# eliasandronicou/split-learning-k8s

Hardware: AMD Instinct MI355X
Metric: training samples/sec (node) for split CNN (higher is better)
Workload: dtype fp32; 1 GPU; K2: split CNN (model_def.py ModelPartA+ModelPartB) both stages fused on 1xMI355X, synthetic 1x28x28 MNIST-shape batches, fp32, HIP-graph step; global_batch=4096, per_gpu_batch=4096, topology=fused-1gpu, graph=True, conv=x3, cut_handoff=client conv1 writes the x3 split input images (slk_conv1_fwd_x3); no f32 cut, client_backward=fused into the x3 dgrad (slk_conv2_dgrad_x3_c1w); no cut gradient in HBM

## Files before the change

include/slk.h:

```cpp
#ifndef SLK_H
#define SLK_H

#include <stdint.h>

#ifdef __cplusplus
extern "C" {
#endif

#define SLK_ABI_VERSION 1

#define SLK_CLIENT_NPARAM 320
#define SLK_SERVER_NPARAM 110666
#define SLK_OFF_W2 0
#define SLK_OFF_B2 18432
#define SLK_OFF_W3 18496
#define SLK_OFF_B3 110656

int slk_abi_version(void);
const char* slk_error_string(int err);
const char* slk_build_id(void);


int slk_conv1_fwd(const float* x, const float* W1, const float* b1, float* act, int B, void* stream);

int slk_conv1_fwd_amax(const float* x, const float* W1, const float* b1, float* act, float* act_amax, int B,
                       void* stream);

int slk_conv1_wgrad(const float* x, const float* act, const float* cut_grad, float* slabs, int B,
                    void* stream);
int slk_conv1_wgrad_nslab(int B);
int slk_conv1_wgrad_remask(const float* x, const float* W1, const float* b1, const float* cut_grad, float* slabs,
                           int B, void* stream);


int slk_conv2_fwd_pool(const float* act, const float* W2, const float* b2, float* pooled,
                       uint8_t* code, int B, void* stream);
int slk_conv2_fwd_pool_direct(const float* act, const float* W2, const float* b2, float* pooled,
                              uint8_t* code, int B, void* stream);

int slk_fc_fwd(const float* pooled, const float* W3, const float* b3, float* logits, int B,
               void* stream);

int slk_xent_fwd_bwd(const float* logits, const int64_t* labels, float* loss_i, float* dlogits,
                     float grad_scale, int* err_flag, int B, void* stream);

int slk_fc_logits_xent(const float* pooled, const float* W3, const float* b3, const int64_t* labels, float* logits,
                       float* loss_i, float* dlogits, float grad_scale, int* err_flag, int B, void* stream);

int slk_fc_dgrad(const float* dlogits, const float* W3, float* dpooled, int B, void* stream);
int slk_fc_dgrad_amax(const float* dlogits, const float* W3, float* dpooled, float* dp_amax, int B, void* stream);

int slk_fc_xent(const float* pooled, const float* W3, const float* b3, const int64_t* labels,
                float* logits, float* loss_i, float* dlogits, float* dpooled, float grad_scale,
                int* err_flag, int B, void* stream);

int slk_fc_xent_amax(const float* pooled, const float* W3, const float* b3, const int64_t* labels, float* logits,
                     float* loss_i, float* dlogits, float* dpooled, float* dp_amax, float grad_scale, int* err_flag,
                     int B, void* stream);


int slk_xent_soft_fwd_bwd(const float* logits, const int64_t* labels, float* loss_i, float* dlogits, float grad_scale,
                          float smoothing, int* err_flag, int B, void* stream);
int slk_fc_logits_xent_soft(const float* pooled, const float* W3, const float* b3, const int64_t* labels,
                            float* logits, float* loss_i, float* dlogits, float grad_scale, float smoothing,
                            int* err_flag, int B, void* stream);
int slk_fc_xent_soft(const float* pooled, const float* W3, const float* b3, const int64_t* labels, float* logits,
                     float* loss_i, float* dlogits, float* dpooled, float* dp_amax, float grad_scale, float smoothing,
                     int* err_flag, int B, void* stream);

int slk_fc_wgrad(const float* dlogits, const float* pooled, float* slabs, int B, void* stream);
int slk_fc_wgrad_nslab(int B);

int slk_conv2_dgrad(const float* dpooled, const uint8_t* code, const float* W2, float* cut_grad,
                    int B, void* stream);
int slk_conv2_dgrad_direct(const float* dpooled, const uint8_t* code, const float* W2, float* cut_grad,
                           int B, void* stream);

int slk_conv2_wgrad(const float* act, const float* dpooled, const uint8_t* code, float* slabs,
                    int B, void* stream);
int slk_conv2_wgrad_nslab(int B);
int slk_conv2_wgrad_direct(const float* act, const float* dpooled, const uint8_t* code, float* slabs,
                           int B, void* stream);
int slk_conv2_wgrad_direct_nslab(int B);


int slk_row_amax(const float* x, int rows, int n, float* amax, void* stream);
int slk_conv2_fwd_pool_x3(const float* act, const float* act_amax, const float* W2, const float* b2, float* pooled,
                          uint8_t* code, int B, void* stream);
int slk_conv2_dgrad_x3(const float* dpooled, const float* dp_amax, const uint8_t* code, const float* W2,
                       float* cut_grad, int B, void* stream);
int slk_conv2_wgrad_x3(const float* act, const float* act_amax, const float* dpooled, const float* dp_amax,
                       const uint8_t* code, float* slabs, int B, void* stream);
int slk_conv2_wgrad_x3_nslab(int B);
int slk_conv2_fwd_pool_x3s(const float* act, const float* act_amax, const float* W2, const float* b2, float* pooled,
                           uint8_t* code, uint16_t* act16, int B, void* stream);
int slk_conv2_wgrad_x3s(const uint16_t* act16, const float* act_amax, const float* dpooled, const float* dp_amax,
                        const uint8_t* code, float* slabs, int B, void* stream);
int slk_conv2_wgrad_x3_form(void);
int slk_mfma_probe_blocks(void);
int slk_mfma_probe(float* out, int iters, void* stream);
int slk_conv2_fwd_pool_x3sa(const float* act, float* act_amax, const float* W2, const float* b2, float* pooled,
                            uint8_t* code, uint16_t* act16, int B, void* stream);
int64_t slk_conv2_act16_bytes(int B);

int slk_conv1_fwd_x3(const float* x, const float* W1, const float* b1, float* act, float* act_amax, uint16_t* act16,
                     uint32_t* relu_bits, int B, void* stream);
int64_t slk_relu_bits_bytes(int B);
int slk_conv2_fwd_pool_x3i(const uint16_t* act16, const float* act_amax, const float* W2, const float* b2,
                           float* pooled, uint8_t* code, int B, void* stream);

int slk_conv2_fwd_pool_x3p(const uint16_t* act16, const float* act_amax, const float* W2, const float* b2,
                           float* pooled, int B, void* stream);

int slk_conv2_dgrad_x3_c1w(const float* dpooled, const float* dp_amax, const uint8_t* code, const float* W2,
                           const float* x, const uint32_t* relu_bits, float* client_slabs, int B, void* stream);
int slk_conv2_dgrad_x3_c1w_nslab(int B);


int slk_fc_eval(const float* pooled, const float* W3, const float* b3, const int64_t* labels, float* logits,
                float* loss_i, int64_t* pred, int* err_flag, int B, void* stream);

int slk_eval_logits(const float* logits, const int64_t* labels, int B, float* loss_i, int64_t* pred, int* err_flag,
                    void* stream);

// ... 171 lines not shown
```

split-learning-k8s_amd/csrc/slk_server.hip:

```cpp
#include "slk_common.h"
#include "slk_eval.h"

using namespace slk;

constexpr int C2F_WAVES = 12;
constexpr int C2F_THREADS = C2F_WAVES * 64;
constexpr int C2F_IMG = 16 * A_PIX;
constexpr int C2F_WH = 72 * 2 * 64;
constexpr int C2F_TPW = 3;
constexpr int C2F_GRID = 256;
constexpr int C2F_CHUNKS = (C2F_IMG * 4 + 1023) / 1024;

typedef __attribute__((address_space(3))) void* lds_ptr_t;

__device__ __forceinline__ void c2f_dma_half(const float* __restrict__ src, float* dst, int wave, int lane) {
    const char* s = reinterpret_cast<const char*>(src);
    char* d = reinterpret_cast<char*>(dst);
    for (int c = wave; c < C2F_CHUNKS; c += C2F_WAVES) {
        const int off = c * 1024 + lane * 16;
        if (off < C2F_IMG * 4)
            __builtin_amdgcn_global_load_lds((const void*)(s + off), (lds_ptr_t)(d + c * 1024), 16, 0, 0);
    }
}

// ... 596 lines not shown
        __syncthreads();
    }

    if constexpr ((MODE & 4) != 0) {
        const float4* W34 = reinterpret_cast<const float4*>(W3);
        float4* D4 = reinterpret_cast<float4*>(dpooled + (size_t)s0 * P_SAMPLE);
        float dmx[FCH_S];
#pragma unroll
        for (int s = 0; s < FCH_S; ++s) dmx[s] = 0.f;
        for (int k4 = tid; k4 < FC_K4; k4 += FCH_T) {
            asm volatile("" ::: "memory");
            float4 w[NCLS];
#pragma unroll
            for (int jj = 0; jj < NCLS; ++jj) w[jj] = W34[jj * FC_K4 + k4];
#pragma unroll
            for (int s = 0; s < FCH_S; ++s) {
                if (s < ns) {
                    float4 o = make_float4(0.f, 0.f, 0.f, 0.f);
#pragma unroll
                    for (int jj = 0; jj < NCLS; ++jj) {
                        const float d = dl[s][jj];
                        o.x = fmaf(d, w[jj].x, o.x);
                        o.y = fmaf(d, w[jj].y, o.y);
                        o.z = fmaf(d, w[jj].z, o.z);
                        o.w = fmaf(d, w[jj].w, o.w);
                    }
                    D4[s * FC_K4 + k4] = o;
                    dmx[s] = fmaxf(dmx[s], fmaxf(fmaxf(fabsf(o.x), fabsf(o.y)), fmaxf(fabsf(o.z), fabsf(o.w))));
                }
            }
        }
        if (dp_amax) {
#pragma unroll
            for (int s = 0; s < FCH_S; ++s) {
                const float v = wave_max(dmx[s]);
                if (lane == 0) mx[wave][s] = v;
            }
            __syncthreads();
            if (tid < ns) {
                float v = mx[0][tid];
#pragma unroll
                for (int w = 1; w < FCH_W; ++w) v = fmaxf(v, mx[w][tid]);
                dp_amax[s0 + tid] = v;
            }
        }
    }
}

#ifndef SLK_FCW_MAXSPLIT
#define SLK_FCW_MAXSPLIT 64
#endif
constexpr int FCW_MAXSPLIT = SLK_FCW_MAXSPLIT;
constexpr int FCW_SLAB = W3_N + NCLS;
__global__ __launch_bounds__(256) void fc_wgrad_kernel(const float* __restrict__ dlogits,
                                                       const float* __restrict__ pooled,
                                                       float* __restrict__ slabs, int B, int per) {
    const int k4 = blockIdx.x * 256 + threadIdx.x;
    const int sp = blockIdx.y;
    const int bs = sp * per, be = min(B, bs + per);
    float4 acc[NCLS];
#pragma unroll
    for (int jj = 0; jj < NCLS; ++jj) acc[jj] = make_float4(0.f, 0.f, 0.f, 0.f);
    const float4* P4 = reinterpret_cast<const float4*>(pooled);
    int b = bs;
    for (; b + 8 <= be; b += 8) {
        float4 p[8];
#pragma unroll
        for (int u = 0; u < 8; ++u) p[u] = P4[(size_t)(b + u) * FC_K4 + k4];
#pragma unroll
        for (int u = 0; u < 8; ++u)
#pragma unroll
            for (int jj = 0; jj < NCLS; ++jj) {
                const float d = dlogits[(b + u) * NCLS + jj];
                acc[jj].x = fmaf(d, p[u].x, acc[jj].x); acc[jj].y = fmaf(d, p[u].y, acc[jj].y);
                acc[jj].z = fmaf(d, p[u].z, acc[jj].z); acc[jj].w = fmaf(d, p[u].w, acc[jj].w);
            }
    }
    for (; b < be; ++b) {
        const float4 p = P4[(size_t)b * FC_K4 + k4];
#pragma unroll
        for (int jj = 0; jj < NCLS; ++jj) {
            const float d = dlogits[b * NCLS + jj];
            acc[jj].x = fmaf(d, p.x, acc[jj].x); acc[jj].y = fmaf(d, p.y, acc[jj].y);
            acc[jj].z = fmaf(d, p.z, acc[jj].z); acc[jj].w = fmaf(d, p.w, acc[jj].w);
        }
    }
    float* slab = slabs + (size_t)sp * FCW_SLAB;
#pragma unroll
    for (int jj = 0; jj < NCLS; ++jj) reinterpret_cast<float4*>(slab + jj * P_SAMPLE)[k4] = acc[jj];
    if (blockIdx.x == 0 && threadIdx.x < NCLS) {
        float s = 0.f;
        for (int bb = bs; bb < be; ++bb) s += dlogits[bb * NCLS + threadIdx.x];
        slab[W3_N + threadIdx.x] = s;
    }
}

static inline int fcw_per(int B) {
    int ns = (B + 63) / 64;
    if (ns > FCW_MAXSPLIT) ns = FCW_MAXSPLIT;
    if (ns < 1) ns = 1;
    return (B + ns - 1) / ns;
}
extern "C" int slk_fc_wgrad_nslab(int B) {
    if (B <= 0) return 0;
    const int per = fcw_per(B);
    return (B + per - 1) / per;
}

extern "C" int slk_conv2_fwd_pool_direct(const float* act, const float* W2, const float* b2, float* pooled,
                                  uint8_t* code, int B, void* stream) {
    SLK_CHECK_ARG(B >= 0);
    if (B == 0) return 0;
    SLK_CHECK_ARG(act && W2 && b2 && pooled && code);
    conv2_fwd_pool_kernel<<<B < C2F_GRID ? B : C2F_GRID, C2F_THREADS, 0, slk_stream(stream)>>>(
        act, W2, b2, pooled, code, B);
    return slk_launch_status();
}

extern "C" int slk_conv2_dgrad_direct(const float* dpooled, const uint8_t* code, const float* W2,
                               float* cut_grad, int B, void* stream) {
    SLK_CHECK_ARG(B >= 0);
    if (B == 0) return 0;
    SLK_CHECK_ARG(dpooled && code && W2 && cut_grad);
    conv2_dgrad_kernel<<<B < C2D_GRID ? B : C2D_GRID, C2D_THREADS, 0, slk_stream(stream)>>>(
        dpooled, code, W2, cut_grad, B);
    return slk_launch_status();
}

extern "C" int slk_conv2_wgrad_direct(const float* act, const float* dpooled, const uint8_t* code,
                               float* slabs, int B, void* stream) {
    SLK_CHECK_ARG(B >= 0);
    if (B == 0) return 0;
    SLK_CHECK_ARG(act && dpooled && code && slabs);
    conv2_wgrad_kernel<<<slk_conv2_wgrad_direct_nslab(B), C2W_THREADS, 0, slk_stream(stream)>>>(
        act, dpooled, code, slabs, B);
    return slk_launch_status();
}

extern "C" int slk_fc_fwd(const float* pooled, const float* W3, const float* b3, float* logits,
                          int B, void* stream) {
    SLK_CHECK_ARG(B >= 0);
    if (B == 0) return 0;
    SLK_CHECK_ARG(pooled && W3 && b3 && logits);
    fc_head16_kernel<1><<<(B + FCH_S - 1) / FCH_S, FCH_T, 0, slk_stream(stream)>>>(
        pooled, W3, b3, nullptr, logits, nullptr, nullptr, nullptr, 0.f, nullptr, B, nullptr);
    return slk_launch_status();
}

extern "C" int slk_xent_fwd_bwd(const float* logits, const int64_t* labels, float* loss_i,
                                float* dlogits, float grad_scale, int* err_flag, int B, void* stream) {
    SLK_CHECK_ARG(B >= 0);
    if (B == 0) return 0;
    SLK_CHECK_ARG(logits && labels && loss_i && dlogits);
    fc_head16_kernel<2><<<(B + FCH_S - 1) / FCH_S, FCH_T, 0, slk_stream(stream)>>>(
        nullptr, nullptr, nullptr, labels, const_cast<float*>(logits), loss_i, dlogits, nullptr,
        grad_scale, err_flag, B, nullptr);
    return slk_launch_status();
}

extern "C" int slk_fc_logits_xent(const float* pooled, const float* W3, const float* b3, const int64_t* labels,
                                  float* logits, float* loss_i, float* dlogits, float grad_scale, int* err_flag, int B,
// ... 58 lines not shown
    fc_head16_kernel<7><<<(B + FCH_S - 1) / FCH_S, FCH_T, 0, slk_stream(stream)>>>(
        pooled, W3, b3, labels, logits, loss_i, dlogits, dpooled, grad_scale, err_flag, B, dp_amax);
    return slk_launch_status();
}

#define SLK_CHECK_SMOOTHING(e) SLK_CHECK_ARG((e) >= 0.f && (e) <= 1.f)

extern "C" int slk_xent_soft_fwd_bwd(const float* logits, const int64_t* labels, float* loss_i, float* dlogits,
                                     float grad_scale, float smoothing, int* err_flag, int B, void* stream) {
    SLK_CHECK_ARG(B >= 0);
    SLK_CHECK_SMOOTHING(smoothing);
    if (B == 0) return 0;
    SLK_CHECK_ARG(logits && labels && loss_i && dlogits);
    fc_head16_kernel<2, true><<<(B + FCH_S - 1) / FCH_S, FCH_T, 0, slk_stream(stream)>>>(
        nullptr, nullptr, nullptr, labels, const_cast<float*>(logits), loss_i, dlogits, nullptr, grad_scale, err_flag, B,
        nullptr, nullptr, smoothing);
    return slk_launch_status();
}

extern "C" int slk_fc_logits_xent_soft(const float* pooled, const float* W3, const float* b3, const int64_t* labels,
                                       float* logits, float* loss_i, float* dlogits, float grad_scale, float smoothing,
                                       int* err_flag, int B, void* stream) {
    SLK_CHECK_ARG(B >= 0);
    SLK_CHECK_SMOOTHING(smoothing);
    if (B == 0) return 0;
    SLK_CHECK_ARG(pooled && W3 && b3 && labels && logits && loss_i && dlogits);
    fc_head16_kernel<3, true><<<(B + FCH_S - 1) / FCH_S, FCH_T, 0, slk_stream(stream)>>>(
        pooled, W3, b3, labels, logits, loss_i, dlogits, nullptr, grad_scale, err_flag, B, nullptr, nullptr, smoothing);
    return slk_launch_status();
}

extern "C" int slk_fc_xent_soft(const float* pooled, const float* W3, const float* b3, const int64_t* labels,
                                float* logits, float* loss_i, float* dlogits, float* dpooled, float* dp_amax,
                                float grad_scale, float smoothing, int* err_flag, int B, void* stream) {
    SLK_CHECK_ARG(B >= 0);
    SLK_CHECK_SMOOTHING(smoothing);
    if (B == 0) return 0;
    SLK_CHECK_ARG(pooled && W3 && b3 && labels && logits && loss_i && dlogits && dpooled);
    fc_head16_kernel<7, true><<<(B + FCH_S - 1) / FCH_S, FCH_T, 0, slk_stream(stream)>>>(
        pooled, W3, b3, labels, logits, loss_i, dlogits, dpooled, grad_scale, err_flag, B, dp_amax, nullptr, smoothing);
    return slk_launch_status();
}

extern "C" int slk_fc_wgrad(const float* dlogits, const float* pooled, float* slabs, int B,
                            void* stream) {
    SLK_CHECK_ARG(B >= 0);
    if (B == 0) return 0;
    SLK_CHECK_ARG(dlogits && pooled && slabs);
    const int per = fcw_per(B);
    dim3 grid(FC_K4 / 256, (B + per - 1) / per);
    fc_wgrad_kernel<<<grid, 256, 0, slk_stream(stream)>>>(dlogits, pooled, slabs, B, per);
    return slk_launch_status();
}
```

split-learning-k8s_amd/splitcnn/_lib.py:

```python
from __future__ import annotations

import ctypes
import os

import torch

from .build import CSRC_DIR, LIB_PATH, source_hash

_c_float_p = ctypes.c_void_p
_P = ctypes.c_void_p
_I = ctypes.c_int
_F = ctypes.c_float
_U = ctypes.c_uint
_L = ctypes.c_int64

_SIGS = {
    "slk_abi_version": [],
    "slk_cut_blocks": [_L],
    "slk_cut_encode": [_P, _L, _P, _P, _P, _P, _P, _P],
    "slk_cut_offsets": [_P, _L, _P, _P, _P, _P],
    "slk_cut_pack": [_P, _L, _P, _P, _P, _P],
    "slk_cut_unpack": [_P, _L, _P, _P, _P, _P],
    "slk_cut_ranks": [_P, _L, _P, _P, _P],
    "slk_cut_unpack_x3": [_P, _P, _P, _P, _I, _P, _P],
    "slk_conv2_dgrad_x3_pack": [_P, _P, _P, _P, _P, _P, _P, _I, _P],
    "slk_cut_offsets_ranks_parts": [_P, _I, _L, _P],
    "slk_cut_unpack_x3_parts": [_P, _I, _P, _I, _P, _P],
    "slk_conv2_dgrad_x3_pack_parts": [_P, _P, _P, _P, _P, _I, _I, _P],
    "slk_error_string": [_I],
    "slk_build_id": [],
    "slk_conv1_fwd": [_P, _P, _P, _P, _I, _P],
    "slk_conv1_fwd_amax": [_P, _P, _P, _P, _P, _I, _P],
    "slk_conv1_wgrad": [_P, _P, _P, _P, _I, _P],
    "slk_conv1_wgrad_nslab": [_I],
    "slk_conv1_wgrad_remask": [_P, _P, _P, _P, _P, _I, _P],
    "slk_conv2_fwd_pool": [_P, _P, _P, _P, _P, _I, _P],
    "slk_conv2_fwd_pool_direct": [_P, _P, _P, _P, _P, _I, _P],
    "slk_fc_fwd": [_P, _P, _P, _P, _I, _P],
    "slk_xent_fwd_bwd": [_P, _P, _P, _P, _F, _P, _I, _P],
    "slk_fc_logits_xent": [_P, _P, _P, _P, _P, _P, _P, _F, _P, _I, _P],
    "slk_fc_dgrad": [_P, _P, _P, _I, _P],
    "slk_fc_dgrad_amax": [_P, _P, _P, _P, _I, _P],
    "slk_fc_xent": [_P, _P, _P, _P, _P, _P, _P, _P, _F, _P, _I, _P],
    "slk_fc_xent_amax": [_P, _P, _P, _P, _P, _P, _P, _P, _P, _F, _P, _I, _P],
    "slk_xent_soft_fwd_bwd": [_P, _P, _P, _P, _F, _F, _P, _I, _P],
    "slk_fc_logits_xent_soft": [_P, _P, _P, _P, _P, _P, _P, _F, _F, _P, _I, _P],
    "slk_fc_xent_soft": [_P, _P, _P, _P, _P, _P, _P, _P, _P, _F, _F, _P, _I, _P],
    "slk_wide_head_soft": [_P, _P, _P, _P, _P, _U, _U, _F, _F, _F, _P, _P, _P, _P, _P, _P, _P, _I, _I, _P],
    "slk_image_batch_mix": [_P, _P, _I, _I, _I, _I, _P, _P, _I, _P, _P, _I, _I, _U, _U, ctypes.c_double, _P, _P, _P,
                            _P],
    "slk_fc_wgrad": [_P, _P, _P, _I, _P],
    "slk_fc_wgrad_nslab": [_I],
    "slk_conv2_dgrad": [_P, _P, _P, _P, _I, _P],
    "slk_conv2_dgrad_direct": [_P, _P, _P, _P, _I, _P],
    "slk_conv2_wgrad": [_P, _P, _P, _P, _I, _P],
    "slk_conv2_wgrad_nslab": [_I],
    "slk_conv2_wgrad_direct": [_P, _P, _P, _P, _I, _P],
    "slk_conv2_wgrad_direct_nslab": [_I],
    "slk_row_amax": [_P, _I, _I, _P, _P],
    "slk_conv2_fwd_pool_x3": [_P, _P, _P, _P, _P, _P, _I, _P],
    "slk_conv2_dgrad_x3": [_P, _P, _P, _P, _P, _I, _P],
    "slk_conv2_wgrad_x3": [_P, _P, _P, _P, _P, _P, _I, _P],
    "slk_conv2_wgrad_x3_nslab": [_I],
    "slk_conv2_fwd_pool_x3s": [_P, _P, _P, _P, _P, _P, _P, _I, _P],
    "slk_conv2_fwd_pool_x3sa": [_P, _P, _P, _P, _P, _P, _P, _I, _P],
    "slk_mfma_probe": [_P, _I, _P],
    "slk_mfma_probe_blocks": [],
    "slk_conv2_wgrad_x3s": [_P, _P, _P, _P, _P, _P, _I, _P],
    "slk_conv2_wgrad_x3_form": [],
    "slk_conv2_act16_bytes": [_I],
    "slk_conv1_fwd_x3": [_P, _P, _P, _P, _P, _P, _P, _I, _P],
    "slk_relu_bits_bytes": [_I],
    "slk_conv2_fwd_pool_x3i": [_P, _P, _P, _P, _P, _P, _I, _P],
    "slk_conv2_fwd_pool_x3p": [_P, _P, _P, _P, _P, _I, _P],
    "slk_fc_eval": [_P, _P, _P, _P, _P, _P, _P, _P, _I, _P],
    "slk_eval_logits": [_P, _P, _I, _P, _P, _P, _P],
    "slk_eval_accumulate": [_P, _P, _P, _I, _P, _P],
    "slk_conv2_dgrad_x3_c1w": [_P, _P, _P, _P, _P, _P, _P, _I, _P],
    "slk_conv2_dgrad_x3_c1w_nslab": [_I],
    "slk_reduce_slabs": [_P, _I, _I, _P, _I, _P],
    "slk_sgd_from_slabs": [_P, _P, _P, _I, _I, _F, _P],
    "slk_sgd": [_P, _P, _I, _F, _P],
    "slk_loss_sum": [_P, _I, _F, _P, _P],
    "slk_loss_log": [_P, _I, _F, _P, _I, _P, _P],
    "slk_sgd_multi_from_slabs": [_P, _P, _P, _P, _P, _I, _F, _P, _I, _F, _P, _I, _P, _P],
    "slk_sgdm_from_slabs": [_P, _P, _P, _P, _I, _I, _P, _I, _P, _F, _F, _F, _I, _P],
    "slk_sgdm_multi_from_slabs": [_P, _P, _P, _P, _P, _P, _I, _P, _I, _P, _F, _F, _F, _I, _P, _I, _F, _P, _I, _P,
                                  _P],
    "slk_reduce_sqnorm_nblk": [_I, _I],
    "slk_reduce_sqnorm_multi": [_P, _P, _P, _P, _P, _I, _P, _I, _P, _I, _F, _P, _I, _P, _P],
    "slk_sgdm_clip_multi": [_P, _P, _P, _P, _P, _P, _I, _P, _P, _I, _P, _P, _I, _P, _F, _F, _F, _I, _P],
    "slk_adamw_clip_multi": [_P, _P, _P, _P, _P, _P, _P, _I, _P, _P, _I, _P, _P, _I, _P, _F, _F, _F, _F, _I, _P],
    "slk_reduce_tnorm_multi": [_P, _P, _P, _P, _P, _P, _P, _I, _P, _I, _P, _I, _F, _P, _I, _P, _P],
    "slk_lars_multi": [_P, _P, _P, _P, _P, _P, _P, _I, _P, _P, _I, _P, _I, _P, _F, _F, _F, _I, _F, _F, _I, _P],
    "slk_lamb_moments_multi": [_P, _P, _P, _P, _P, _P, _P, _P, _P, _I, _P, _I, _P, _F, _F, _F, _F, _I, _P, _I, _F,
                               _P, _I, _P, _P],
    "slk_lamb_multi": [_P, _P, _P, _P, _P, _P, _P, _I, _P, _P, _I, _P, _I, _P, _F, _F, _F, _F, _I, _P],
    "slk_ema_multi": [_P, _P, _P, _I, _P, _P, _I, _I, _P],
    "slk_cut8_encode": [_P, _I, _I, _P, _P],
    "slk_cut8_decode": [_P, _I, _I, _P, _P, _P],
    "slk_cut8_roundtrip": [_P, _I, _I, _P, _P],
    "slk_cut8_record_bytes": [],
    "slk_mnist_batch": [_P, _P, _I, _P, _I, _F, _F, _P, _P, _P, _P],
    "slk_image_batch": [_P, _P, _I, _I, _I, _I, _P, _I, _P, _P, _I, _I, _U, _U, _P, _P, _P, _P],
    "slk_wide_conv1_fwd": [_P, _P, _P, _P, _P, _I, _P],
# ... 88 lines not shown
```

split-learning-k8s_amd/splitcnn/engine.py:

```python
from __future__ import annotations

import contextlib
from collections import defaultdict
from typing import Callable, Dict, List, Optional, Tuple

import torch
import torch.nn as nn

from . import ops
from .graphs import GraphedTrainer
from .loss import LABEL_ERROR, SoftCrossEntropy, check_loss
from .model_def import ModelPartA, ModelPartB
from .optim import EMA, LARS, SGD, ClipNorm, LRSchedule, check_clip, check_ema, is_layerwise

LR = 0.01


class KernelTimer:

    def __init__(self):
        self.enabled = False
        self._ev: Dict[str, list] = defaultdict(list)

    @contextlib.contextmanager
# ... 288 lines not shown

    def step_from_slabs(self, slabs: torch.Tensor) -> None:
        with TIMER("sgd_client"):
            if self.optim is None:
                ops.sgd_from_slabs(self.params, self.grads, slabs, self.lr)
            else:
                self._sgdm([(0, ops.CLIENT_NPARAM, slabs)])
                self._tick()

    def backward(self, cut_grad: torch.Tensor, x: Optional[torch.Tensor] = None,
                 act: Optional[torch.Tensor] = None, accumulate: bool = False) -> None:
        slabs = self._slabs(cut_grad, x, act)
        ops.reduce_slabs(slabs, out=self.grads, accumulate=accumulate)

    def step(self):
        with TIMER("sgd_client"):
            if self.optim is None:
                ops.sgd(self.params, self.grads, self.lr)
            else:
                self._sgdm([(self.params, None, self.buf, self.grads.view(1, -1))])
                self._tick()


class ServerStage(_SgdRecipe):

    PAIRS = ((0, ops.CONV2_SLAB, 18432), (ops.CONV2_SLAB, ops.SERVER_NPARAM, 92160))
    TENSORS = ("conv2.weight", "conv2.bias", "fc1.weight", "fc1.bias")

    def __init__(self, model: Optional[ModelPartB] = None, lr: float = LR, device="cuda",
                 loss_log: Optional[LossLog] = None, conv: str = CONV_DEFAULT,
                 optim: Optional[SGD] = None, schedule: Optional[LRSchedule] = None,
                 clip: Optional[ClipNorm] = None, loss: Optional[SoftCrossEntropy] = None,
                 ema: Optional[EMA] = None):
        self.device = torch.device(device)
        self.loss = check_loss(loss)
        self.conv = conv
        self.impl_fwd, self.impl_dgrad, self.impl_wgrad = CONV_PRESETS[conv]
        self.share_images = True
        self.model = (model if model is not None else ModelPartB()).to(self.device)
        self.lr = lr
        m = self.model
        self.params, self.grads = _flatten_params(
            [m.conv2.weight, m.conv2.bias, m.fc1.weight, m.fc1.bias], self.device)
        self._init_optim(lr, optim, schedule, clip, ema)
        self.loss_log = loss_log if loss_log is not None else LossLog(self.device)
        self.err_flag = torch.zeros(1, dtype=torch.int32, device=self.device)
        self.eval_err_flag = torch.zeros(1, dtype=torch.int32, device=self.device)
        self.eval_logits = None
        self.fuse_optim = True
        self.fc_wgrad_early = False
        self.wgrad_first = False
        self.fc_split = True
        self.fc_one_launch = True
        self._buf = _Buffers()

    def bind_grads(self, view: torch.Tensor):
        view.copy_(self.grads)
        self.grads = view
        m = self.model
        m.conv2.weight.grad = view[:18432].view(64, 32, 3, 3)
        m.conv2.bias.grad = view[18432:18496].view(64)
        m.fc1.weight.grad = view[18496:110656].view(10, 9216)
        m.fc1.bias.grad = view[110656:].view(10)

    def _b(self, name, shape, dtype=torch.float32):
        return self._buf.get(name, shape, dtype, self.device)

    def forward_backward(self, act: Optional[torch.Tensor], labels: torch.Tensor, grad_scale: float,
                         cut_grad: Optional[torch.Tensor] = None, act_amax: Optional[torch.Tensor] = None,
                         act16: Optional[torch.Tensor] = None, client_fuse=None, cut_pack=None):
        B = labels.shape[0]
        m = self.model
        W2, b2 = m.conv2.weight.detach(), m.conv2.bias.detach()
        W3, b3 = m.fc1.weight.detach(), m.fc1.bias.detach()
        fi, di, wi = self.impl_fwd, self.impl_dgrad, self.impl_wgrad
        if act16 is not None and ((fi, wi) != ("x3", "x3") or act_amax is None):
            raise ValueError("act16 input needs the x3 forward and wgrad (conv preset 'x3') and act_amax")
        if act_amax is None and "x3" in (fi, wi):
            with TIMER("act_amax"):
                act_amax = ops.row_amax(act, out=self._b("act_amax", (B,)))
        dp_amax = self._b("dp_amax", (B,)) if "x3" in (di, wi) else None
        pooled_b, code_b = self._b("pooled", (B, 64, 12, 12)), self._b("code", (B, 64, 12, 12), torch.uint8)
        if act16 is not None:
            with TIMER("conv2_fwd_pool"):
                pooled, code = ops.conv2_fwd_pool_x3i(act16, act_amax, W2, b2, pooled=pooled_b, code=code_b)
        else:
            act16 = (self._b("act16", (ops.conv2_act16_bytes(B),), torch.uint8)
                     if fi == "x3" and wi == "x3" and self.share_images else None)
            with TIMER("conv2_fwd_pool"):
                pooled, code = ops.conv2_fwd_pool(act, W2, b2, pooled=pooled_b, code=code_b, impl=fi,
                                                  act_amax=act_amax, act16=act16)
        split = self.fc_split and dp_amax is not None
        soft = None if self.loss is None else float(self.loss.label_smoothing)
        if split:
            with TIMER("fc_xent"):
                if self.fc_one_launch and soft is None:
                    _, loss_i, dlogits = ops.fc_logits_xent(
                        pooled, W3, b3, labels, grad_scale, logits=self._b("logits", (B, 10)),
                        loss_i=self._b("loss_i", (B,)), dlogits=self._b("dlogits", (B, 10)), err_flag=self.err_flag)
                elif self.fc_one_launch:
                    _, loss_i, dlogits = ops.fc_logits_xent_soft(
                        pooled, W3, b3, labels, grad_scale, soft, logits=self._b("logits", (B, 10)),
                        loss_i=self._b("loss_i", (B,)), dlogits=self._b("dlogits", (B, 10)), err_flag=self.err_flag)
                else:
                    logits = ops.fc_fwd(pooled, W3, b3, out=self._b("logits", (B, 10)))
                    if soft is None:
                        loss_i, dlogits = ops.xent_fwd_bwd(logits, labels, grad_scale, loss_i=self._b("loss_i", (B,)),
                                                           dlogits=self._b("dlogits", (B, 10)), err_flag=self.err_flag)
                    else:
                        loss_i, dlogits = ops.xent_soft_fwd_bwd(
                            logits, labels, grad_scale, soft, loss_i=self._b("loss_i", (B,)),
                            dlogits=self._b("dlogits", (B, 10)), err_flag=self.err_flag)
            with TIMER("fc_wgrad"):
                s3 = ops.fc_wgrad_slabs(dlogits, pooled, slabs=self._b("s3", (ops.fc_wgrad_nslab(B), ops.FC_SLAB)))
            dpooled = self._b("dpooled", (B, 64, 12, 12))
            with TIMER("fc_dgrad"):
                ops.fc_dgrad(dlogits, W3, out=dpooled.view(B, 9216), dp_amax=dp_amax)
        else:
            with TIMER("fc_xent"):
                if soft is None:
                    _, loss_i, dlogits, dpooled = ops.fc_xent(
                        pooled, W3, b3, labels, grad_scale, logits=self._b("logits", (B, 10)),
                        loss_i=self._b("loss_i", (B,)), dlogits=self._b("dlogits", (B, 10)),
                        dpooled=self._b("dpooled", (B, 64, 12, 12)), err_flag=self.err_flag, dp_amax=dp_amax)
                else:
                    _, loss_i, dlogits, dpooled = ops.fc_xent_soft(
                        pooled, W3, b3, labels, grad_scale, soft, logits=self._b("logits", (B, 10)),
                        loss_i=self._b("loss_i", (B,)), dlogits=self._b("dlogits", (B, 10)),
                        dpooled=self._b("dpooled", (B, 64, 12, 12)), err_flag=self.err_flag, dp_amax=dp_amax)
        if self.fc_wgrad_early and not split:
            with TIMER("fc_wgrad"):
                s3 = ops.fc_wgrad_slabs(dlogits, pooled, slabs=self._b("s3", (ops.fc_wgrad_nslab(B), ops.FC_SLAB)))

        def wgrad():
            with TIMER("conv2_wgrad"):
                return ops.conv2_wgrad_slabs(act, dpooled, code,
                                             slabs=self._b("s2", (ops.conv2_wgrad_nslab(B, impl=wi), ops.CONV2_SLAB)),
                                             impl=wi, act_amax=act_amax, dp_amax=dp_amax, act16=act16)
        if self.wgrad_first:
            s2 = wgrad()
        if cut_pack is not None:
            if di != "x3":
                raise ValueError("cut_pack needs the x3 dgrad (conv preset 'x3' or 'x3w')")
            with TIMER("conv2_dgrad"):
                ops.conv2_dgrad_x3_pack_parts(dpooled, code, W2, dp_amax, *cut_pack)
            cut_grad = None
        elif client_fuse is not None:
            if di != "x3":
                raise ValueError("client_fuse needs the x3 dgrad (conv preset 'x3' or 'x3w')")
            cx, cbits, cslabs = client_fuse
            with TIMER("conv2_dgrad"):
                ops.conv2_dgrad_client_slabs(dpooled, code, W2, cx, cbits, dp_amax=dp_amax, slabs=cslabs)
            cut_grad = None
        else:
            if cut_grad is None:
                cut_grad = self._b("cut_grad", (B, 32, 26, 26))
            with TIMER("conv2_dgrad"):
                ops.conv2_dgrad(dpooled, code, W2, out=cut_grad, impl=di, dp_amax=dp_amax)
        if not self.wgrad_first:
            s2 = wgrad()
        if not self.fc_wgrad_early and not split:
            with TIMER("fc_wgrad"):
                s3 = ops.fc_wgrad_slabs(dlogits, pooled, slabs=self._b("s3", (ops.fc_wgrad_nslab(B), ops.FC_SLAB)))
        return cut_grad, loss_i, s2, s3

    def apply_grad_slabs(self, s2, s3):
        with TIMER("sgd_server"):
            if self.optim is None:
                ops.sgd_from_slabs(self.params[:ops.CONV2_SLAB], self.grads[:ops.CONV2_SLAB], s2, self.lr)
                ops.sgd_from_slabs(self.params[ops.CONV2_SLAB:], self.grads[ops.CONV2_SLAB:], s3, self.lr)
# ... 172 lines not shown
```

split-learning-k8s_amd/splitcnn/ops.py:

```python
from __future__ import annotations

import ctypes

import torch

from . import _lib

CLIENT_NPARAM = 320
SERVER_NPARAM = 110666
OFF_W2, OFF_B2, OFF_W3, OFF_B3 = 0, 18432, 18496, 110656
CONV2_SLAB = 18496
FC_SLAB = 92170

_F32 = torch.float32


def _stream(t: torch.Tensor) -> int:
    return torch.cuda.current_stream(t.device).cuda_stream


def _dev(t: torch.Tensor, name: str, shape=None, dtype=_F32) -> int:
    if not isinstance(t, torch.Tensor):
        raise TypeError(f"{name}: expected a torch.Tensor")
    if t.device.type != "cuda":
# ... 282 lines not shown


def xent_soft_fwd_bwd(logits, labels, grad_scale, smoothing, loss_i=None, dlogits=None, err_flag=None):
    B = batch_of(logits, (10,), "logits")
    loss_i = _out(loss_i, (B,), logits, name="loss_i")
    dlogits = _out(dlogits, (B, 10), logits, name="dlogits")
    eptr = _dev(err_flag, "err_flag", (1,), torch.int32) if err_flag is not None else None
    _lib.call("slk_xent_soft_fwd_bwd", _dev(logits, "logits"), _labels(labels, B), _dev(loss_i, "loss_i"),
              _dev(dlogits, "dlogits"), float(grad_scale), float(smoothing), eptr, B, _stream(logits))
    return loss_i, dlogits


def fc_logits_xent_soft(pooled, W3, b3, labels, grad_scale, smoothing, logits=None, loss_i=None, dlogits=None,
                        err_flag=None):
    B = _pooled_batch(pooled)
    logits = _out(logits, (B, 10), pooled, name="logits")
    loss_i = _out(loss_i, (B,), pooled, name="loss_i")
    dlogits = _out(dlogits, (B, 10), pooled, name="dlogits")
    eptr = _dev(err_flag, "err_flag", (1,), torch.int32) if err_flag is not None else None
    _lib.call("slk_fc_logits_xent_soft", _dev(pooled, "pooled"), _dev(W3, "fc1.weight", (10, 9216)),
              _dev(b3, "fc1.bias", (10,)), _labels(labels, B), _dev(logits, "logits"), _dev(loss_i, "loss_i"),
              _dev(dlogits, "dlogits"), float(grad_scale), float(smoothing), eptr, B, _stream(pooled))
    return logits, loss_i, dlogits


def fc_xent_soft(pooled, W3, b3, labels, grad_scale, smoothing, logits=None, loss_i=None, dlogits=None,
                 dpooled=None, err_flag=None, dp_amax=None):
    B = _pooled_batch(pooled)
    logits = _out(logits, (B, 10), pooled, name="logits")
    loss_i = _out(loss_i, (B,), pooled, name="loss_i")
    dlogits = _out(dlogits, (B, 10), pooled, name="dlogits")
    dpooled = _out(dpooled, tuple(pooled.shape), pooled, name="dpooled")
    eptr = _dev(err_flag, "err_flag", (1,), torch.int32) if err_flag is not None else None
    _lib.call("slk_fc_xent_soft", _dev(pooled, "pooled"), _dev(W3, "fc1.weight", (10, 9216)),
              _dev(b3, "fc1.bias", (10,)), _labels(labels, B), _dev(logits, "logits"), _dev(loss_i, "loss_i"),
              _dev(dlogits, "dlogits"), _dev(dpooled, "dpooled"),
              _dev(dp_amax, "dp_amax", (B,)) if dp_amax is not None else None, float(grad_scale), float(smoothing),
              eptr, B, _stream(pooled))
    return logits, loss_i, dlogits, dpooled


def fc_wgrad_nslab(B: int) -> int:
    return _lib.query("slk_fc_wgrad_nslab", B)


def fc_wgrad_slabs(dlogits, pooled, slabs=None):
    B = batch_of(dlogits, (10,), "dlogits")
    if _pooled_batch(pooled) != B:
        raise ValueError("pooled / dlogits batch mismatch")
    slabs = _out(slabs, (fc_wgrad_nslab(B), FC_SLAB), dlogits, name="slabs")
    _lib.call("slk_fc_wgrad", _dev(dlogits, "dlogits"), _dev(pooled, "pooled"), _dev(slabs, "slabs"),
              B, _stream(dlogits))
    return slabs


def _dpooled_batch(dpooled):
    return _pooled_batch(dpooled)


def conv2_dgrad(dpooled, code, W2, out=None, direct=False, impl=None, dp_amax=None):
    impl = _impl(direct, impl)
    B = _dpooled_batch(dpooled)
    cut_grad = _out(out, (B, 32, 26, 26), dpooled, name="cut_grad")
    if impl == "x3":
        if dp_amax is None:
            dp_amax = row_amax(dpooled)
        _lib.call("slk_conv2_dgrad_x3", _dev(dpooled, "dpooled"), _dev(dp_amax, "dp_amax", (B,)),
                  _dev(code, "code", (B, 64, 12, 12), torch.uint8), _dev(W2, "conv2.weight", (64, 32, 3, 3)),
                  _dev(cut_grad, "cut_grad"), B, _stream(dpooled))
        return cut_grad
    direct = impl == "direct"
    _lib.call("slk_conv2_dgrad_direct" if direct else "slk_conv2_dgrad", _dev(dpooled, "dpooled"),
              _dev(code, "code", (B, 64, 12, 12), torch.uint8), _dev(W2, "conv2.weight", (64, 32, 3, 3)),
              _dev(cut_grad, "cut_grad"), B, _stream(dpooled))
    return cut_grad


def conv2_dgrad_x3_pack(dpooled, code, W2, dp_amax, mask, ranks, vals):
    B = _dpooled_batch(dpooled)
    nw = (B * 21632 + 31) // 32
    _lib.call("slk_conv2_dgrad_x3_pack", _dev(dpooled, "dpooled"), _dev(dp_amax, "dp_amax", (B,)),
              _dev(code, "code", (B, 64, 12, 12), torch.uint8), _dev(W2, "conv2.weight", (64, 32, 3, 3)),
              _dev(mask, "mask", (nw,), torch.int32), _dev(ranks, "ranks", (nw,), torch.int32),
              _dev(vals, "vals"), B, _stream(dpooled))
    return vals


def conv2_dgrad_x3_pack_parts(dpooled, code, W2, dp_amax, parts, part_b):
    B = _dpooled_batch(dpooled)
    if part_b <= 0 or B % part_b:
        raise ValueError(f"part_b {part_b} must divide the chunk's {B} samples")
    _lib.call("slk_conv2_dgrad_x3_pack_parts", _dev(dpooled, "dpooled"), _dev(dp_amax, "dp_amax", (B,)),
              _dev(code, "code", (B, 64, 12, 12), torch.uint8), _dev(W2, "conv2.weight", (64, 32, 3, 3)),
              _dev(parts, "parts", (B // part_b, 3), torch.int64), part_b, B, _stream(dpooled))


def cut_unpack_x3_parts(parts, part_b, act_amax, act16):
    B = batch_of(act_amax, (), "act_amax")
    if part_b <= 0 or B % part_b:
        raise ValueError(f"part_b {part_b} must divide the chunk's {B} samples")
    _lib.call("slk_cut_unpack_x3_parts", _dev(parts, "parts", (B // part_b, 3), torch.int64), part_b,
              _dev(act_amax, "act_amax", (B,)), B, _act16(act16, B), _stream(act_amax))
    return act16


def cut_offsets_ranks_parts(parts, n):
# ... 441 lines not shown
```

Measured before the change: 5.222 million samples/s.

## Fuse FC weight-gradient and data-gradient into one heterogeneous-block launch

Adds an fc_backward kernel whose first blocks run the FC weight-gradient slab reduction and whose remaining blocks compute dpooled = dlogits·W3 plus the per-row abs-max, all from a single launch. The weight-gradient path now reads pooled with nontemporal loads to avoid polluting cache. The dgrad part register-prefetches the next W3 tile and batches eight samples per block. The goal is to remove one launch and let the two independent reductions share the GPU concurrently inside the graph, at the cost of a more complex kernel whose two block types may be imbalanced.

```diff
diff --git a/include/slk.h b/include/slk.h
--- a/include/slk.h
+++ b/include/slk.h
@@ -70,6 +70,9 @@
 
 int slk_fc_wgrad(const float* dlogits, const float* pooled, float* slabs, int B, void* stream);
 int slk_fc_wgrad_nslab(int B);
+
+int slk_fc_backward(const float* dlogits, const float* W3, const float* pooled, float* dpooled, float* dp_amax,
+                    float* slabs, int B, void* stream);
 
 int slk_conv2_dgrad(const float* dpooled, const uint8_t* code, const float* W2, float* cut_grad,
                     int B, void* stream);
diff --git a/split-learning-k8s_amd/csrc/slk_server.hip b/split-learning-k8s_amd/csrc/slk_server.hip
--- a/split-learning-k8s_amd/csrc/slk_server.hip
+++ b/split-learning-k8s_amd/csrc/slk_server.hip
@@ -672,11 +672,20 @@
 #endif
 constexpr int FCW_MAXSPLIT = SLK_FCW_MAXSPLIT;
 constexpr int FCW_SLAB = W3_N + NCLS;
-__global__ __launch_bounds__(256) void fc_wgrad_kernel(const float* __restrict__ dlogits,
-                                                       const float* __restrict__ pooled,
-                                                       float* __restrict__ slabs, int B, int per) {
-    const int k4 = blockIdx.x * 256 + threadIdx.x;
-    const int sp = blockIdx.y;
+template <bool NT>
+__device__ __forceinline__ float4 fcw_ld(const float4* p) {
+    if constexpr (NT) {
+        typedef float f4v __attribute__((ext_vector_type(4)));
+        const f4v v = __builtin_nontemporal_load(reinterpret_cast<const f4v*>(p));
+        return make_float4(v.x, v.y, v.z, v.w);
+    } else {
+        return *p;
+    }
+}
+template <bool NT = false>
+__device__ __forceinline__ void fcw_block(const float* __restrict__ dlogits, const float* __restrict__ pooled,
+                                          float* __restrict__ slabs, int B, int per, int cb, int sp) {
+    const int k4 = cb * 256 + threadIdx.x;
     const int bs = sp * per, be = min(B, bs + per);
     float4 acc[NCLS];
 #pragma unroll
@@ -686,7 +695,7 @@
     for (; b + 8 <= be; b += 8) {
         float4 p[8];
 #pragma unroll
-        for (int u = 0; u < 8; ++u) p[u] = P4[(size_t)(b + u) * FC_K4 + k4];
+        for (int u = 0; u < 8; ++u) p[u] = fcw_ld<NT>(P4 + (size_t)(b + u) * FC_K4 + k4);
 #pragma unroll
         for (int u = 0; u < 8; ++u)
 #pragma unroll
@@ -697,7 +706,7 @@
             }
     }
     for (; b < be; ++b) {
-        const float4 p = P4[(size_t)b * FC_K4 + k4];
+        const float4 p = fcw_ld<NT>(P4 + (size_t)b * FC_K4 + k4);
 #pragma unroll
         for (int jj = 0; jj < NCLS; ++jj) {
             const float d = dlogits[b * NCLS + jj];
@@ -708,11 +717,17 @@
     float* slab = slabs + (size_t)sp * FCW_SLAB;
 #pragma unroll
     for (int jj = 0; jj < NCLS; ++jj) reinterpret_cast<float4*>(slab + jj * P_SAMPLE)[k4] = acc[jj];
-    if (blockIdx.x == 0 && threadIdx.x < NCLS) {
+    if (cb == 0 && threadIdx.x < NCLS) {
         float s = 0.f;
         for (int bb = bs; bb < be; ++bb) s += dlogits[bb * NCLS + threadIdx.x];
         slab[W3_N + threadIdx.x] = s;
     }
+}
+
+__global__ __launch_bounds__(256) void fc_wgrad_kernel(const float* __restrict__ dlogits,
+                                                       const float* __restrict__ pooled,
+                                                       float* __restrict__ slabs, int B, int per) {
+    fcw_block(dlogits, pooled, slabs, B, per, blockIdx.x, blockIdx.y);
 }
 
 static inline int fcw_per(int B) {
@@ -727,6 +742,81 @@
     return (B + per - 1) / per;
 }
 
+constexpr int FCB_T = 256, FCB_S = 8, FCB_W = FCB_T / 64, FCB_TRIPS = FC_K4 / FCB_T;
+static_assert(FC_K4 % FCB_T == 0 && FCB_S * NCLS <= FCB_T, "fc backward tiling");
+
+__global__ __launch_bounds__(FCB_T) void fc_backward_kernel(
+    const float* __restrict__ dlogits, const float* __restrict__ W3, const float* __restrict__ pooled,
+    float* __restrict__ dpooled, float* __restrict__ dp_amax, float* __restrict__ slabs, int B, int per,
+    unsigned nw) {
+    if (blockIdx.x < nw) {
+        const unsigned w = blockIdx.x;
+        fcw_block<true>(dlogits, pooled, slabs, B, per, (int)(w % (FC_K4 / 256)), (int)(w / (FC_K4 / 256)));
+        return;
+    }
+    const unsigned d0 = blockIdx.x - nw;
+    __shared__ __attribute__((aligned(16))) float dl[NCLS][FCB_S];
+    __shared__ float mx[FCB_W][FCB_S];
+    const int tid = threadIdx.x, lane = tid & 63;
+    const int wave = __builtin_amdgcn_readfirstlane(tid >> 6);
+    const int s0 = (int)d0 * FCB_S;
+    const int ns = min(FCB_S, B - s0);
+    const float4* W34 = reinterpret_cast<const float4*>(W3);
+    float4* D4 = reinterpret_cast<float4*>(dpooled + (size_t)s0 * P_SAMPLE);
+    float4 w[NCLS];
+#pragma unroll
+    for (int jj = 0; jj < NCLS; ++jj) w[jj] = W34[jj * FC_K4 + tid];
+    if (tid < FCB_S * NCLS) {
+        const int s = tid / NCLS, jj = tid - s * NCLS;
+        dl[jj][s] = s < ns ? dlogits[(size_t)(s0 + s) * NCLS + jj] : 0.f;
+    }
+    __syncthreads();
+    float dmx[FCB_S];
+#pragma unroll
+    for (int s = 0; s < FCB_S; ++s) dmx[s] = 0.f;
+#pragma unroll 1
+    for (int t = 0; t < FCB_TRIPS; ++t) {
+        const float4* Wn = W34 + (t + 1 < FCB_TRIPS ? t + 1 : t) * FCB_T;
+        float4* Dt = D4 + t * FCB_T;
+        float4 o[FCB_S];
+#pragma unroll
+        for (int s = 0; s < FCB_S; ++s) o[s] = make_float4(0.f, 0.f, 0.f, 0.f);
+#pragma unroll
+        for (int jj = 0; jj < NCLS; ++jj) {
+            asm volatile("" ::: "memory");
+            const float4 wj = w[jj];
+            w[jj] = Wn[jj * FC_K4 + tid];
+#pragma unroll
+            for (int s = 0; s < FCB_S; ++s) {
+                const float d = dl[jj][s];
+                o[s].x = fmaf(d, wj.x, o[s].x);
+                o[s].y = fmaf(d, wj.y, o[s].y);
+                o[s].z = fmaf(d, wj.z, o[s].z);
+                o[s].w = fmaf(d, wj.w, o[s].w);
+            }
+        }
+#pragma unroll
+        for (int s = 0; s < FCB_S; ++s) asm volatile("" : "+v"(o[s].x), "+v"(o[s].y), "+v"(o[s].z), "+v"(o[s].w));
+#pragma unroll
+        for (int s = 0; s < FCB_S; ++s) {
+            if (s < ns) Dt[s * FC_K4 + tid] = o[s];
+            dmx[s] = fmaxf(dmx[s], fmaxf(fmaxf(fabsf(o[s].x), fabsf(o[s].y)), fmaxf(fabsf(o[s].z), fabsf(o[s].w))));
+        }
+    }
+#pragma unroll
+    for (int s = 0; s < FCB_S; ++s) {
+        const float v = wave_max(dmx[s]);
+        if (lane == 0) mx[wave][s] = v;
+    }
+    __syncthreads();
+    if (tid < ns) {
+        float v = mx[0][tid];
+#pragma unroll
+        for (int ww = 1; ww < FCB_W; ++ww) v = fmaxf(v, mx[ww][tid]);
+        dp_amax[s0 + tid] = v;
+    }
+}
+
 extern "C" int slk_conv2_fwd_pool_direct(const float* act, const float* W2, const float* b2, float* pooled,
                                   uint8_t* code, int B, void* stream) {
     SLK_CHECK_ARG(B >= 0);
@@ -891,3 +981,15 @@
     fc_wgrad_kernel<<<grid, 256, 0, slk_stream(stream)>>>(dlogits, pooled, slabs, B, per);
     return slk_launch_status();
 }
+
+extern "C" int slk_fc_backward(const float* dlogits, const float* W3, const float* pooled, float* dpooled,
+                               float* dp_amax, float* slabs, int B, void* stream) {
+    SLK_CHECK_ARG(B >= 0);
+    if (B == 0) return 0;
+    SLK_CHECK_ARG(dlogits && W3 && pooled && dpooled && dp_amax && slabs);
+    const int per = fcw_per(B);
+    const unsigned nd = (unsigned)((B + FCB_S - 1) / FCB_S), nw = (unsigned)((FC_K4 / 256) * ((B + per - 1) / per));
+    fc_backward_kernel<<<nd + nw, FCB_T, 0, slk_stream(stream)>>>(dlogits, W3, pooled, dpooled, dp_amax, slabs, B, per,
+                                                                  nw);
+    return slk_launch_status();
+}
diff --git a/split-learning-k8s_amd/splitcnn/_lib.py b/split-learning-k8s_amd/splitcnn/_lib.py
--- a/split-learning-k8s_amd/splitcnn/_lib.py
+++ b/split-learning-k8s_amd/splitcnn/_lib.py
@@ -51,6 +51,7 @@
                             _P],
     "slk_fc_wgrad": [_P, _P, _P, _I, _P],
     "slk_fc_wgrad_nslab": [_I],
+    "slk_fc_backward": [_P, _P, _P, _P, _P, _P, _I, _P],
     "slk_conv2_dgrad": [_P, _P, _P, _P, _I, _P],
     "slk_conv2_dgrad_direct": [_P, _P, _P, _P, _I, _P],
     "slk_conv2_wgrad": [_P, _P, _P, _P, _I, _P],
diff --git a/split-learning-k8s_amd/splitcnn/engine.py b/split-learning-k8s_amd/splitcnn/engine.py
--- a/split-learning-k8s_amd/splitcnn/engine.py
+++ b/split-learning-k8s_amd/splitcnn/engine.py
@@ -364,6 +364,7 @@
         self.wgrad_first = False
         self.fc_split = True
         self.fc_one_launch = True
+        self.fc_backward_one_launch = True
         self._buf = _Buffers()
 
     def bind_grads(self, view: torch.Tensor):
@@ -423,11 +424,16 @@
                         loss_i, dlogits = ops.xent_soft_fwd_bwd(
                             logits, labels, grad_scale, soft, loss_i=self._b("loss_i", (B,)),
                             dlogits=self._b("dlogits", (B, 10)), err_flag=self.err_flag)
-            with TIMER("fc_wgrad"):
-                s3 = ops.fc_wgrad_slabs(dlogits, pooled, slabs=self._b("s3", (ops.fc_wgrad_nslab(B), ops.FC_SLAB)))
+            s3 = self._b("s3", (ops.fc_wgrad_nslab(B), ops.FC_SLAB))
             dpooled = self._b("dpooled", (B, 64, 12, 12))
-            with TIMER("fc_dgrad"):
-                ops.fc_dgrad(dlogits, W3, out=dpooled.view(B, 9216), dp_amax=dp_amax)
+            if self.fc_backward_one_launch:
+                with TIMER("fc_backward"):
+                    ops.fc_backward(dlogits, W3, pooled, dpooled=dpooled.view(B, 9216), dp_amax=dp_amax, slabs=s3)
+            else:
+                with TIMER("fc_wgrad"):
+                    ops.fc_wgrad_slabs(dlogits, pooled, slabs=s3)
+                with TIMER("fc_dgrad"):
+                    ops.fc_dgrad(dlogits, W3, out=dpooled.view(B, 9216), dp_amax=dp_amax)
         else:
             with TIMER("fc_xent"):
                 if soft is None:
diff --git a/split-learning-k8s_amd/splitcnn/ops.py b/split-learning-k8s_amd/splitcnn/ops.py
--- a/split-learning-k8s_amd/splitcnn/ops.py
+++ b/split-learning-k8s_amd/splitcnn/ops.py
@@ -358,6 +358,18 @@
     _lib.call("slk_fc_wgrad", _dev(dlogits, "dlogits"), _dev(pooled, "pooled"), _dev(slabs, "slabs"),
               B, _stream(dlogits))
     return slabs
+
+
+def fc_backward(dlogits, W3, pooled, dpooled=None, dp_amax=None, slabs=None):
+    B = batch_of(dlogits, (10,), "dlogits")
+    if _pooled_batch(pooled) != B:
+        raise ValueError("pooled / dlogits batch mismatch")
+    dpooled = _out(dpooled, (B, 9216), dlogits, name="dpooled")
+    dp_amax = _out(dp_amax, (B,), dlogits, name="dp_amax")
+    slabs = _out(slabs, (fc_wgrad_nslab(B), FC_SLAB), dlogits, name="slabs")
+    _lib.call("slk_fc_backward", _dev(dlogits, "dlogits"), _dev(W3, "fc1.weight", (10, 9216)), _dev(pooled, "pooled"),
+              _dev(dpooled, "dpooled"), _dev(dp_amax, "dp_amax", (B,)), _dev(slabs, "slabs"), B, _stream(dlogits))
+    return dpooled, dp_amax, slabs
 
 
 def _dpooled_batch(dpooled):
```

Result: faster. 5.293 million samples/s (median of 6 runs) (+1.4%).
